# Duy1230/Map-Reduced-Approach-for-Vietnamese-Long-Document-Summarization

Hardware: AMD Instinct MI355X
Metric: map-phase chunks/sec (2k-tok chunk, 256-tok summary) at 1/2/4/8 MI355X (higher is better)
Workload: dtype f16

## Files before the change

### include/mapsum.h

```cpp
#ifndef MAPSUM_H
#define MAPSUM_H

#include <stddef.h>
#include <stdint.h>

#ifdef __cplusplus
extern "C" {
#endif

#define MS_ABI_VERSION 3

#define MS_OK 0
#define MS_EIO -5
#define MS_ENOMEM -12
#define MS_EBUSY -16
#define MS_EINVAL -22
#define MS_ENOSPC -28

#define MS_FINISH_EOS 1
#define MS_FINISH_LENGTH 2
#define MS_FINISH_ERROR 3

#define MS_FLAG_IGNORE_EOS 1u

// ... 67 lines not shown
                     const void* host_blocks, int64_t n_bytes);
int ms_init_synthetic_q(ms_engine* e, uint64_t seed, float scale, float norm_jitter);

int ms_weight_regions(const ms_engine* e, void** ptrs, int64_t* bytes, int32_t cap);
int ms_quant_manifest(const ms_engine* e, int32_t* triples, int32_t cap);
int ms_declare_weight_q(ms_engine* e, int32_t tensor, int32_t layer, int32_t ggml_type);

int ms_submit(ms_engine* e, const int32_t* ids, int32_t n, int32_t num_predict,
              uint32_t flags, uint64_t tag);
#define MS_SAMPLE_MAX_TOPK 256
#define MS_SAMPLE_MAX_WINDOW 256
typedef struct ms_sampling {
  float temperature;
  int32_t top_k;
  float top_p;
  float min_p;
  float repeat_penalty;
  int32_t repeat_last_n;
  uint64_t seed;
} ms_sampling;
int ms_submit_sampled(ms_engine* e, const int32_t* ids, int32_t n, int32_t num_predict,
                      uint32_t flags, uint64_t tag, const ms_sampling* sp);
int ms_set_eos_ids(ms_engine* e, const int32_t* ids, int32_t n);
int ms_step(ms_engine* e);
int ms_poll(ms_engine* e, ms_result* out, int32_t cap);
int ms_pending(const ms_engine* e);
int ms_get_stats(const ms_engine* e, ms_stats* out);
int ms_reset_stats(ms_engine* e);
int ms_set_profiling(ms_engine* e, uint32_t class_mask);
int ms_trace_push(const char* name);
int ms_trace_pop(void);
int ms_synchronize(ms_engine* e);
int ms_set_persist(ms_engine* e, int32_t on);
#define MS_DBG_KPOOL 0
#define MS_DBG_VPOOL 1
#define MS_DBG_DECODE_LOGITS 2
#define MS_DBG_DECODE_X 3
#define MS_DBG_PREFILL_LOGITS 4
int ms_debug_read(ms_engine* e, int32_t which, int64_t offset, void* host, int64_t bytes);
int ms_debug_pk_stamps(uint64_t* out, int32_t n);
int ms_debug_a2_stamps(uint64_t* out, int32_t n);

int ms_forward(ms_engine* e, const int32_t* ids, int32_t n, int32_t n_layers_run,
               float* hidden_out, float* logits_out);
int ms_forward_packed(ms_engine* e, const int32_t* ids, const int32_t* lens, int32_t n_seqs,
                      int32_t n_layers_run, float* hidden_out, float* logits_out);
int ms_submit_forced(ms_engine* e, const int32_t* ids, int32_t n, const int32_t* forced,
                     int32_t n_forced, int32_t num_predict, uint32_t flags, uint64_t tag);

#define MS_EPI_STORE_F16 0
#define MS_EPI_ADD_F32 1
#define MS_EPI_SWIGLU 2
#define MS_EPI_STORE_F32 3
#define MS_EPI_ARGMAX 5
int ms_op_gemm(const void* A, const void* W, void* out, int32_t M, int32_t N, int32_t K,
               int32_t ldo, int32_t epilogue, void* stream);
int ms_op_gemm_resid(const void* A, const void* W, float* x, void* xg_out, const void* gamma, float* ssq_out,
                     int32_t M, int32_t N, int32_t K, void* stream);
int ms_gemm_resid_tiles(int32_t M, int32_t N);
int ms_set_gemm_variant(int32_t variant);
int ms_set_qgemv_gs(int32_t on);
int ms_set_attn_tuning(int32_t combine_grp, int32_t order);
int ms_set_dgemm_kh(int32_t kh);
int ms_set_dgemm_wn(int32_t wn);
int64_t ms_op_gemv_workspace(int32_t M, int32_t N, int32_t K);
int ms_op_gemv(const void* X, const void* W, void* out, int32_t M, int32_t N, int32_t K,
// ... 36 lines not shown
```

### map-reduced-approach-for-vietnamese-long-document-summarization_amd/csrc/engine.cpp

```cpp
#include <hip/hip_runtime.h>

#include <algorithm>
#include <cmath>
#include <cstddef>
#include <cstdio>
#include <cstdlib>
#include <cstring>
#include <deque>
#include <array>
#include <functional>
#include <map>
#include <tuple>
#include <memory>
#include <stdexcept>
#include <string>
#include <vector>

#if MS_HAVE_ROCTX
#include <rocprofiler-sdk-roctx/roctx.h>
#else
static inline int roctxRangePushA(const char*) { return 0; }
static inline int roctxRangePop() { return 0; }
#endif

// ... 142 lines not shown
  }
  bool large(int) const { return large_engine && (!has_quant || cfg.max_batch >= qlarge_min); }
  bool qd(const QSlot* q, int M, int N, int K, int S, int epi) const {
    if (!qdgemm_mode || !q || !q->ready()) return false;
    const QMat& m = q->m;
    const bool q4 = m.type0 == MS_QT_Q4_K && (m.n < 2 || m.type1 == MS_QT_Q4_K) && (m.n < 3 || m.type2 == MS_QT_Q4_K);
    return (q4 || qdgemm_mode == 2) && qdgemm_supported(M, N, K, S, epi, m);
  }
  bool row_groups(int B) const { return !large(B) && B > kMaxGemvRows; }
  int qsplit = 4;
  bool attn_slabs = true;
  RowScale cur_rs{};
  int32_t* args_d = nullptr;
  int32_t* args_h = nullptr;
  size_t args_cap = 0;
  struct Ctx {
    hipStream_t stream = nullptr;
    float* x = nullptr;
    float* ssq = nullptr;
    f16_t *xb = nullptr, *qkv = nullptr, *attn = nullptr, *hbuf = nullptr;
    float* logits = nullptr;
    int32_t* ids_out_d = nullptr;
    int32_t* args_d = nullptr;
    int32_t* args_h = nullptr;
    size_t args_cap = 0;
    hipEvent_t ev_a = nullptr, ev_b = nullptr;
  } cp, cd;
  bool overlap = false;
  void use(const Ctx& c) {
    stream = c.stream; x = c.x; ssq = c.ssq; xb = c.xb; qkv = c.qkv; attn = c.attn; hbuf = c.hbuf;
    logits = c.logits; ids_out_d = c.ids_out_d; args_d = c.args_d; args_h = c.args_h;
    args_cap = c.args_cap; ev_a = c.ev_a; ev_b = c.ev_b;
  }
  std::vector<uint8_t> stop_set;
  std::deque<std::unique_ptr<Seq>> waiting;
  std::vector<std::unique_ptr<Seq>> running;
  std::vector<std::unique_ptr<Seq>> done, polled;
  ms_stats stats{};
  uint32_t prof_mask = 0;
  std::vector<std::pair<int, int>> ev_pending;
  size_t ev_used = 0;
  hipEvent_t ev_a = nullptr, ev_b = nullptr;
  std::map<std::tuple<int, int, int, int>, std::pair<hipGraphExec_t, uint64_t>> decode_graphs;
  uint64_t graph_clock = 0;
  static constexpr size_t kMaxGraphs = 64;
  int graph_steps = 16;
  bool use_graphs = true;
  int32_t* ids_host = nullptr;
  int32_t* first_host = nullptr;
  int32_t* ids_ring_d = nullptr;
  static constexpr int kMaxRun = 64;
  int max_run = kMaxRun;
  SampleSlot* samp_d = nullptr;
  SampleSlot* samp_h = nullptr;
  std::vector<uint8_t> slot_sampled;

  template <class T>
  T* dalloc(size_t n, bool zero = false) {
    void* p = nullptr;
    if (n == 0) n = 1;
    hipError_t e = hipMalloc(&p, n * sizeof(T));
    if (e != hipSuccess)
      throw MsError(MS_ENOMEM, "hipMalloc(" + std::to_string(n * sizeof(T)) + " B) failed: " +
                                   hipGetErrorString(e));
    allocs.push_back(p);
    if (zero) HIP_OK(hipMemset(p, 0, n * sizeof(T)));
// ... 193 lines not shown
      ga.tok_pos = tok_pos;
      ga.tok_slot = tok_slot;
      ga.cos_tab = cos_tab;
      ga.sin_tab = sin_tab;
      ga.kv = kv;
      ga.Hq = Hq;
      ga.Hk = Hk;
      ga.rs = rs_attn;
      proj(&Q[QS_QKV], xb, Ly.wqkv, qkv, B, QKVN, H, QKVN, MS_GEMV_EPI_ROPE_KV, &ga, K_GEMV);
      qa = DecodeQKV{qkv, nullptr, 0, cos_tab, sin_tab, RowScale{}};
    }
    attn_decode(qa, kv, da);
    resid_update(&Q[QS_O], attn, Ly.wo, B, Hq * D, split_o, dsplit_o, Ly.ffn_norm, dwn_o);
    const RowScale rs_ffn = cur_rs;
    const f16_t* g_next = l + 1 < L ? layers[l + 1].attn_norm : final_norm;
    if (large(B)) {
      prof_begin(K_GEMV);
      if (qd(&Q[QS_GU], B, 2 * F, H, 1, MS_GEMV_EPI_SWIGLU))
        launch_qdgemm(xb, Q[QS_GU].m, hbuf, B, 2 * F, H, 1, F, MS_GEMV_EPI_SWIGLU, stream, &rs_ffn);
      else if (qdf(B, 2 * F, H, 1, MS_GEMV_EPI_SWIGLU))
        launch_qdgemm_f16(xb, Ly.wgu, hbuf, B, 2 * F, H, 1, F, MS_GEMV_EPI_SWIGLU, stream, &rs_ffn);
      else
        launch_dgemm(xb, Ly.wgu, hbuf, B, 2 * F, H, 1, F, MS_GEMV_EPI_SWIGLU, stream, &rs_ffn, dgemm_kh);
      prof_end(K_GEMV);
    } else {
      GemvArgs gg{};
      gg.rs = rs_ffn;
      proj(&Q[QS_GU], xb, Ly.wgu, hbuf, B, 2 * F, H, F, MS_GEMV_EPI_SWIGLU, &gg, K_GEMV, sizeof(f16_t));
    }
    resid_update(&Q[QS_DOWN], hbuf, Ly.wdown, B, F, split_down, dsplit_down, g_next, dwn_down);
  }

  void run_layer(int l, int T, bool decode, const int32_t* tok_pos, const int32_t* tok_slot,
                 const PrefillAttnArgs& pa, const DecodeAttnArgs& da, bool tail = true) {
    if (decode && fused_decode(T)) {
      run_layer_fused_decode(l, T, tok_pos, tok_slot, da);
      return;
    }
    const Layer& Ly = layers[l];
    const int kc = decode ? K_GEMV : K_GEMM;
    const RowScale rs_attn = cur_rs;
    KVView kv = kv_layer(l);
    gemm_or_gemv(xb, Ly.wqkv, qkv, T, QKVN, H, QKVN, MS_EPI_STORE_F16, decode, kc, &rs_attn);
    prof_begin(K_MISC);
    launch_rope_kv(qkv, T, Hq, Hk, tok_pos, tok_slot, cos_tab, sin_tab, kv, stream, decode || !pa.cos_tab);
    prof_end(K_MISC);
    if (decode) {
      attn_decode(DecodeQKV{qkv, nullptr, 0, cos_tab, sin_tab, RowScale{}}, kv, da);
    } else {
      prof_begin(K_ATTN_PREFILL);
      launch_attn_prefill(qkv, attn, Hq, Hk, kv, pa, stream);
      prof_end(K_ATTN_PREFILL);
    }
    const f16_t* g_next = l + 1 < L ? layers[l + 1].attn_norm : final_norm;
    if (decode) {
      gemm_or_gemv(attn, Ly.wo, x, T, H, Hq * D, H, MS_EPI_ADD_F32, decode, kc);
      norm_input(Ly.ffn_norm, T);
    } else {
      prefill_resid(attn, Ly.wo, T, Hq * D, Ly.ffn_norm);
    }
    const RowScale rs_ffn = cur_rs;
    gemm_or_gemv(xb, Ly.wgu, hbuf, T, 2 * F, H, F, MS_EPI_SWIGLU, decode, kc, &rs_ffn);
    if (decode) {
      gemm_or_gemv(hbuf, Ly.wdown, x, T, H, F, H, MS_EPI_ADD_F32, decode, kc);
      if (tail) norm_input(g_next, T);
    } else if (tail) {
      prefill_resid(hbuf, Ly.wdown, T, F, g_next);
    } else {
      gemm_or_gemv(hbuf, Ly.wdown, x, T, H, F, H, MS_EPI_ADD_F32, decode, kc);
    }
  }

  bool prefill_resid_ok(int T) const {
    const int tiles = gemm_resid_tiles(T, H);
    return tiles <= kGemmRsTiles && gemm_rs_tiles_ok(T, QKVN, tiles) && gemm_rs_tiles_ok(T, 2 * F, tiles);
  }
  void prefill_resid(const f16_t* X, const f16_t* W, int T, int K, const f16_t* g_next) {
    if (!prefill_resid_ok(T)) {
      gemm_or_gemv(X, W, x, T, H, K, H, MS_EPI_ADD_F32, false, K_GEMM);
      norm_input(g_next, T);
      return;
    }
    GemmResid gr{g_next, xb, ssq};
    prof_begin(K_GEMM);
    launch_gemm(X, W, x, T, H, K, H, MS_EPI_ADD_F32, stream, nullptr, &gr);
    prof_end(K_GEMM);
    cur_rs = make_row_scale(ssq, gemm_resid_tiles(T, H), H, cfg.norm_eps);
  }

  void norm_input(const f16_t* w, int T, const int32_t* row_idx = nullptr) {
    prof_begin(K_MISC);
    launch_rmsnorm(x, w, xb, ssq, T, H, row_idx, stream);
    prof_end(K_MISC);
    cur_rs = norm_rs();
  }

  std::vector<std::array<int32_t, 3>> quant_manifest;
  void note_quant(int tensor, int layer, int type) {
    for (auto& q : quant_manifest)
      if (q[0] == tensor && q[1] == layer) { q[2] = type; return; }
    quant_manifest.push_back({tensor, layer, type});
  }
  std::vector<std::pair<void*, size_t>> weight_regions() const {
    std::vector<std::pair<void*, size_t>> r;
    const size_t H2 = (size_t)H * 2;
    r.push_back({embed, (size_t)V * H2});
    if (!cfg.tie_embeddings) r.push_back({lm_head, (size_t)V * H2});
    r.push_back({final_norm, H2});
    for (const Layer& Ly : layers) {
      r.push_back({Ly.attn_norm, H2});
      r.push_back({Ly.ffn_norm, H2});
      r.push_back({Ly.wqkv, (size_t)QKVN * H2});
      r.push_back({Ly.wo, (size_t)Hq * D * H2});
      r.push_back({Ly.wgu, (size_t)2 * F * H2});
      r.push_back({Ly.wdown, (size_t)F * H2});
    }
    auto qs = [&](const QSlot& q) {
      const uint8_t* b[3] = {q.m.base0, q.m.base1, q.m.base2};
      for (int i = 0; i < 3; ++i)
        if (b[i]) r.push_back({(void*)b[i], q.bytes[i]});
    };
    qs(lmq);
    for (const auto& l : lq)
      for (const QSlot& q : l) qs(q);
    return r;
// ... 127 lines not shown
      Ly.ffn_norm = E.dalloc<f16_t>(E.H);
      Ly.wqkv = E.dalloc<f16_t>((size_t)E.QKVN * E.H);
      Ly.wo = E.dalloc<f16_t>((size_t)E.H * E.Hq * E.D);
      Ly.wgu = E.dalloc<f16_t>((size_t)2 * E.F * E.H);
      Ly.wdown = E.dalloc<f16_t>((size_t)E.H * E.F);
    }
    std::vector<float> cs, sn;
    rope_tables(*cfg, cfg->max_ctx, cs, sn);
    E.cos_tab = E.dalloc<float>(cs.size());
    E.sin_tab = E.dalloc<float>(sn.size());
    HIP_OK(hipMemcpy(E.cos_tab, cs.data(), cs.size() * 4, hipMemcpyHostToDevice));
    HIP_OK(hipMemcpy(E.sin_tab, sn.data(), sn.size() * 4, hipMemcpyHostToDevice));
    E.layer_kv_elems = (size_t)E.n_pages * E.Hk * kPage * E.D;
    E.kpool = E.dalloc<f16_t>(E.layer_kv_elems * E.L, true);
    E.vpool = E.dalloc<f16_t>(E.layer_kv_elems * E.L, true);
    HIP_OK(hipHostMalloc((void**)&E.bt_h, (size_t)cfg->max_batch * E.max_pages * sizeof(int32_t),
                         hipHostMallocDefault));
    std::memset(E.bt_h, 0, (size_t)cfg->max_batch * E.max_pages * sizeof(int32_t));
    E.bt_d = E.dalloc<int32_t>((size_t)cfg->max_batch * E.max_pages, true);
    for (int p = E.n_pages - 1; p >= 0; --p) E.free_pages.push_back(p);
    for (int s = cfg->max_batch - 1; s >= 0; --s) E.free_slots.push_back(s);
    const size_t T = E.Tmax;
    for (ms_engine::Ctx* c : {&E.cp, &E.cd}) {
      const size_t R = c == &E.cp ? T : (size_t)cfg->max_batch;
      c->x = E.dalloc<float>(R * E.H);
      c->ssq = E.dalloc<float>(std::max(R * kGemmRsTiles, (size_t)256 * cfg->max_batch), true);
      c->xb = E.dalloc<f16_t>(R * E.H);
      c->qkv = E.dalloc<f16_t>(R * E.QKVN);
      c->attn = E.dalloc<f16_t>(R * E.Hq * E.D);
      c->hbuf = E.dalloc<f16_t>(R * E.F);
      c->logits = E.dalloc<float>((size_t)cfg->max_batch * E.V);
      c->ids_out_d = E.dalloc<int32_t>(cfg->max_batch);
    }
    const int Md = std::min(cfg->max_batch, 64);
    size_t gws = 0;
    const int shapes[5][2] = {{E.QKVN, E.H}, {E.H, E.Hq * E.D}, {2 * E.F, E.H}, {E.H, E.F}, {E.V, E.H}};
    for (auto& sh : shapes) gws = std::max(gws, gemv_workspace_bytes(Md, sh[0], sh[1]));
    E.gemv_ws = E.dalloc<char>(gws, true);
    E.attn_ppb = attn_decode2_ppb(cfg->max_batch, E.Hk, cfg->max_ctx);
    E.attn_v2 = cfg->max_batch <= 16;
    if (const char* v = getenv("MS_ATTN_V2")) E.attn_v2 = atoi(v) != 0;
    if (const char* v = getenv("MS_ATTN_TICKET")) E.attn_ticket = atoi(v) != 0;
    E.attn_cnt = E.dalloc<unsigned>((size_t)cfg->max_batch * E.Hk, true);
    const int ws_ctx = (cfg->max_ctx + 255) / 256 * 256;
    E.attn_ws = (float*)E.dalloc<char>(std::max(attn_decode_workspace_bytes(cfg->max_batch, E.Hq, ws_ctx),
                                                attn_decode2_workspace_bytes(cfg->max_batch, E.Hq, ws_ctx,
                                                                             E.attn_ppb)),
                                       true);
    E.slabs = E.dalloc<float>((size_t)ms_engine::kMaxSplit * std::min(std::max(cfg->max_batch, 64), 256) *
                              std::max(E.QKVN, E.H));
    if (const char* v = getenv("MS_SPLIT_QKV")) E.split_qkv = atoi(v);
    if (const char* v = getenv("MS_ATTN_SLABS")) E.attn_slabs = atoi(v) != 0;
    if (const char* v = getenv("MS_SPLIT_O")) E.split_o = atoi(v);
    if (const char* v = getenv("MS_SPLIT_DOWN")) E.split_down = atoi(v);
    if (const char* v = getenv("MS_DGEMM_MIN")) E.dgemm_min = atoi(v);
    E.large_engine = cfg->max_batch >= E.dgemm_min;
    if (const char* v = getenv("MS_QLARGE_MIN")) E.qlarge_min = atoi(v);
    if (const char* v = getenv("MS_QDGEMM")) E.qdgemm_mode = atoi(v);
    if (const char* v = getenv("MS_LM_GEMM_MIN")) E.lm_gemm_min = atoi(v);
    E.dgemm_kh = cfg->max_batch <= 128 && E.H % 128 == 0 ? dgemm_kh_setting() : 1;
    if (const char* v = getenv("MS_QDF_MIN")) E.qdf_min = atoi(v);
    if (E.qdf_min > 0 && cfg->max_batch >= E.qdf_min) {
      E.dsplit_qkv = 3;
      E.dsplit_down = 4;
    }
    if (const char* v = getenv("MS_DSPLIT_QKV")) E.dsplit_qkv = atoi(v);
// ... 520 lines not shown
  const size_t o_ids = a.size();
  for (Seq* s : batch) a.insert(a.end(), s->prompt.begin(), s->prompt.end());
  const size_t o_pos = a.size();
  for (Seq* s : batch)
    for (int i = 0; i < (int)s->prompt.size(); ++i) a.push_back(s->len + i);
  const size_t o_slot = a.size();
  for (Seq* s : batch)
    for (int i = 0; i < (int)s->prompt.size(); ++i) a.push_back(s->slot);
  const size_t o_qstart = a.size();
  {
    int q = 0;
    for (Seq* s : batch) { a.push_back(q); q += (int)s->prompt.size(); }
  }
  const size_t o_qlen = a.size();
  for (Seq* s : batch) a.push_back((int)s->prompt.size());
  const size_t o_kvlen = a.size();
  for (Seq* s : batch) a.push_back(s->len + (int)s->prompt.size());
  const size_t o_sslot = a.size();
  for (Seq* s : batch) a.push_back(s->slot);
  const size_t o_last = a.size();
  {
    int q = 0;
    for (Seq* s : batch) { q += (int)s->prompt.size(); a.push_back(q - 1); }
  }
  std::vector<std::pair<int, int32_t>> qb;
  for (int i = 0; i < S; ++i) {
    const int n = (int)batch[i]->prompt.size();
    for (int b = 0; b < (n + kPrefillQRows - 1) / kPrefillQRows; ++b)
      qb.push_back({batch[i]->len + b * kPrefillQRows, (i << 16) | b});
  }
  std::stable_sort(qb.begin(), qb.end(), [](auto& x, auto& y) { return x.first > y.first; });
  const size_t o_qblk = a.size();
  for (auto& p : qb) a.push_back(p.second);
  int32_t* d = E.upload_args(a);

  PrefillAttnArgs pa;
  pa.seq_qstart = d + o_qstart;
  pa.seq_qlen = d + o_qlen;
  pa.seq_kvlen = d + o_kvlen;
  pa.seq_slot = d + o_sslot;
  pa.qblk = d + o_qblk;
  pa.n_qblk = (int)qb.size();
  pa.cos_tab = E.cos_tab;
  pa.sin_tab = E.sin_tab;
  DecodeAttnArgs da{};

  E.prof_begin(K_MISC);
  launch_embed(d + o_ids, T, E.embed, E.H, E.x, E.stream);
  E.prof_end(K_MISC);
  E.norm_input(E.layers[0].attn_norm, T);
  for (int l = 0; l < n_layers_run; ++l)
    E.run_layer(l, T, false, d + o_pos, d + o_slot, pa, da, l + 1 < E.L || logits_all);
  HIP_OK(hipGetLastError());
  if (n_layers_run < E.L) return;
  if (!logits_all && !first_ids) return;
  if (logits_all) {
    launch_gemm(E.xb, E.lm_head, logits_all, T, E.V, E.H, E.V, MS_EPI_STORE_F32, E.stream, &E.cur_rs);
    return;
  }
  E.norm_input(E.final_norm, S, d + o_last);
  for (int r0 = 0; r0 < S; r0 += ms_engine::kMaxGemvRows) {
    const int rows = std::min(S - r0, (int)ms_engine::kMaxGemvRows);
    const RowScale rs = make_row_scale(E.ssq + r0, 1, E.H, E.cfg.norm_eps);
    E.gemm_or_gemv(E.xb + (size_t)r0 * E.H, E.lm_head, E.logits + (size_t)r0 * E.V, rows, E.V, E.H, E.V,
                   MS_EPI_STORE_F32, true, K_LMHEAD, &rs);
  }
  bool samp = false;
  for (Seq* s : batch) samp = samp || s->sampled;
  E.prof_begin(K_MISC);
  if (samp) {
    SampleArgs sa{};
    sa.logits = E.logits;
    sa.ldl = E.V;
    sa.n = E.V;
    sa.slots = E.samp_d;
    sa.row_slot = d + o_sslot;
    sa.ids_out = E.ids_out_d;
    launch_sample_rows(sa, S, E.stream);
  } else {
    launch_argmax(E.logits, S, E.V, E.ids_out_d, E.stream);
  }
  E.prof_end(K_MISC);
  HIP_OK(hipGetLastError());
  first_ids->resize(S);
  HIP_OK(hipMemcpyAsync(E.first_host, E.ids_out_d, S * sizeof(int32_t), hipMemcpyDeviceToHost, E.stream));
}

static void decode_head(ms_engine& E, int B, int32_t* d) {
  E.prof_begin(K_MISC);
  launch_embed(d, B, E.embed, E.H, E.x, E.stream, E.layers[0].attn_norm, E.xb, E.ssq);
  E.prof_end(K_MISC);
}

// ... 356 lines not shown
int ms_trace_pop(void) {
  roctxRangePop();
  return MS_OK;
}

int ms_get_stats(const ms_engine* e, ms_stats* out) {
  if (!e || !out) return MS_EINVAL;
  *out = e->stats;
  return MS_OK;
}

int ms_reset_stats(ms_engine* e) {
  if (!e) return MS_EINVAL;
  e->stats = ms_stats{};
  return MS_OK;
}

int ms_set_profiling(ms_engine* e, uint32_t mask) {
  if (!e) return MS_EINVAL;
  e->prof_mask = mask;
  return MS_OK;
}

int ms_set_persist(ms_engine* e, int32_t on) {
  if (!e) return MS_EINVAL;
  return guarded(e, [&]() -> int {
    HIP_OK(hipStreamSynchronize(e->cd.stream));
    e->persist = on != 0;
    e->drop_graphs();
    return (e->persist_ok ? 1 : 0);
  });
}

int ms_debug_read(ms_engine* e, int32_t which, int64_t offset, void* host, int64_t bytes) {
  if (!e || !host || offset < 0 || bytes < 0) return MS_EINVAL;
  return guarded(e, [&]() -> int {
    ms_engine& E = *e;
    const void* base = nullptr;
    size_t cap = 0;
    switch (which) {
      case MS_DBG_KPOOL: base = E.kpool; cap = E.layer_kv_elems * E.L * sizeof(f16_t); break;
      case MS_DBG_VPOOL: base = E.vpool; cap = E.layer_kv_elems * E.L * sizeof(f16_t); break;
      case MS_DBG_DECODE_LOGITS: base = E.cd.logits; cap = (size_t)E.cfg.max_batch * E.V * sizeof(float); break;
      case MS_DBG_DECODE_X: base = E.cd.x; cap = (size_t)E.cfg.max_batch * E.H * sizeof(float); break;
      case MS_DBG_PREFILL_LOGITS: base = E.cp.logits; cap = (size_t)E.cfg.max_batch * E.V * sizeof(float); break;
      default: REQUIRE(false, MS_EINVAL, "ms_debug_read: unknown buffer");
    }
    REQUIRE((size_t)offset + (size_t)bytes <= cap, MS_EINVAL, "ms_debug_read: range past the buffer");
    HIP_OK(hipStreamSynchronize(E.cd.stream));
    HIP_OK(hipStreamSynchronize(E.cp.stream));
    HIP_OK(hipMemcpy(host, (const char*)base + offset, (size_t)bytes, hipMemcpyDeviceToHost));
    return MS_OK;
  });
}

int ms_debug_pk_stamps(uint64_t* out, int32_t n) {
  if (!out || n < 0) return MS_EINVAL;
  ms::persist_stamps(reinterpret_cast<unsigned long long*>(out), n);
  return MS_OK;
}

int ms_debug_a2_stamps(uint64_t* out, int32_t n) {
  if (!out || n < 0) return MS_EINVAL;
  ms::attn2_stamps(reinterpret_cast<unsigned long long*>(out), n);
  return MS_OK;
}
// ... 381 lines not shown
```

### map-reduced-approach-for-vietnamese-long-document-summarization_amd/csrc/k_misc.hip

```cpp
#include "gemv_common.h"

namespace ms {

thread_local ProfEvents* g_prof = nullptr;

__global__ __launch_bounds__(256) void embed_kernel(const int32_t* __restrict__ ids,
                                                    const f16_t* __restrict__ emb, int H,
                                                    float* __restrict__ x, const f16_t* __restrict__ gamma,
                                                    f16_t* __restrict__ xg, float* __restrict__ ssq) {
  __shared__ float red[4];
  const int t = blockIdx.x;
  const f16_t* row = emb + (size_t)ids[t] * H;
  float* xo = x + (size_t)t * H;
  float ss = 0.f;
  for (int c = threadIdx.x; c < H / 8; c += blockDim.x) {
    uint4 v = *(const uint4*)(row + c * 8);
    const uint32_t w[4] = {v.x, v.y, v.z, v.w};
    float4 a, b;
    a.x = h_lo(w[0]); a.y = h_hi(w[0]);
    a.z = h_lo(w[1]); a.w = h_hi(w[1]);
    b.x = h_lo(w[2]); b.y = h_hi(w[2]);
    b.z = h_lo(w[3]); b.w = h_hi(w[3]);
    *(float4*)(xo + c * 8) = a;
    *(float4*)(xo + c * 8 + 4) = b;
// ... 144 lines not shown
  float4 v[8];
  float ss = 0.f;
#pragma unroll
  for (int k = 0; k < 8; ++k) {
    const int c = min(threadIdx.x + k * 256, n4 - 1);
    v[k] = *(const float4*)(xr + c * 4);
    if (threadIdx.x + k * 256 < n4) ss += v[k].x * v[k].x + v[k].y * v[k].y + v[k].z * v[k].z + v[k].w * v[k].w;
  }
  f16_t* yr = y + (size_t)r * H;
#pragma unroll
  for (int k = 0; k < 8; ++k) {
    const int c = threadIdx.x + k * 256;
    if (c >= n4) break;
    uint2 wv = *(const uint2*)(w + c * 4);
    float g0 = h_lo(wv.x), g1 = h_hi(wv.x);
    float g2 = h_lo(wv.y), g3 = h_hi(wv.y);
    uint2 o;
    o.x = pack2h(v[k].x * g0 * kXgScale, v[k].y * g1 * kXgScale);
    o.y = pack2h(v[k].z * g2 * kXgScale, v[k].w * g3 * kXgScale);
    *(uint2*)(yr + c * 4) = o;
  }
  ss = wave_sum(ss);
  if ((threadIdx.x & 63) == 0) red[threadIdx.x >> 6] = ss;
  __syncthreads();
  if (threadIdx.x == 0) ssq[r] = ((red[0] + red[1]) + red[2]) + red[3];
}

void launch_rmsnorm(const float* x, const f16_t* w, f16_t* y, float* ssq, int rows, int H,
                    const int32_t* row_idx, hipStream_t s) {
  if (rows <= 0) return;
  MS_LAUNCH(rmsnorm_kernel, dim3(rows), dim3(256), 0, s, x, w, y, ssq, H, row_idx);
}

template <int S>
__global__ __launch_bounds__(256) void residual_rmsnorm_kernel(float* __restrict__ x,
                                                               const float* __restrict__ slabs,
                                                               int rows,
                                                               const f16_t* __restrict__ w,
                                                               f16_t* __restrict__ y,
                                                               float* __restrict__ ssq, int H) {
  constexpr int KMAX = 3;
  __shared__ float red[4];
  const int r = blockIdx.x;
  float* xr = x + (size_t)r * H;
  const int n4 = H / 4;
  const size_t slab = (size_t)rows * H;
  typedef uint32_t u32x2 __attribute__((ext_vector_type(2)));
  f32x4 v[KMAX], p[KMAX][S > 0 ? S : 1];
  u32x2 wv[KMAX];
#pragma unroll
  for (int k = 0; k < KMAX; ++k) {
    const int c = min((int)threadIdx.x + k * 256, n4 - 1);
    v[k] = *(const f32x4*)(xr + c * 4);
    wv[k] = *(const u32x2*)(w + c * 4);
#pragma unroll
    for (int q = 0; q < S; ++q) p[k][q] = *(const f32x4*)(slabs + q * slab + (size_t)r * H + c * 4);
  }
  __builtin_amdgcn_sched_barrier(0);
#pragma unroll
  for (int k = 0; k < KMAX; ++k) {
    asm volatile("" : "+v"(v[k]));
    asm volatile("" : "+v"(wv[k]));
#pragma unroll
    for (int q = 0; q < S; ++q) asm volatile("" : "+v"(p[k][q]));
  }
  if constexpr (S > 0) {
// ... 233 lines not shown
```

### map-reduced-approach-for-vietnamese-long-document-summarization_amd/csrc/kernels.h

```cpp
#pragma once
#include "common.h"

namespace ms {

struct KVView {
  f16_t* k;
  f16_t* v;
  const int32_t* block_table;
  int32_t max_pages;
  int32_t n_kv_heads;
  int32_t slot_major;
};

constexpr int kPrefillQRows = 128;
struct PrefillAttnArgs {
  const int32_t* seq_qstart;
  const int32_t* seq_qlen;
  const int32_t* seq_kvlen;
  const int32_t* seq_slot;
  const int32_t* qblk;
  int32_t n_qblk;
  const float* cos_tab;
  const float* sin_tab;
};

struct DecodeAttnArgs {
  const int32_t* seq_len;
  const int32_t* seq_slot;
  int32_t B;
  int32_t max_len;
  int32_t ppw;
};

struct RowScale {
  const float* ssq;
  int tiles, H;
  float eps;
  float inv_h;
};
inline RowScale make_row_scale(const float* ssq, int tiles, int H, float eps) {
  return RowScale{ssq, tiles, H, eps, 1.0f / (float)H};
}
constexpr float kXgScale = 0.0625f, kXgUnscale = 16.0f;
__device__ __forceinline__ float rs_rinv(float sum, const RowScale& rs) {
  return __builtin_amdgcn_rsqf(__fmaf_rn(sum, rs.inv_h, rs.eps)) * kXgUnscale;
}

void launch_embed(const int32_t* ids, int T, const f16_t* emb, int H, float* x, hipStream_t s,
                  const f16_t* gamma = nullptr, f16_t* xg = nullptr, float* ssq = nullptr);
void launch_decode_advance(int32_t* args, const int32_t* ids_out, int32_t* ring, int B, int V,
                           hipStream_t s);
void launch_decode_tail(const void* partials, int tiles, int32_t* args, int32_t* ids_out, int32_t* ring, int B,
                        int V, const f16_t* emb, int H, float* x, const f16_t* gamma, f16_t* xg, float* ssq,
                        hipStream_t s);
void launch_rmsnorm(const float* x, const f16_t* w, f16_t* y, float* ssq, int rows, int H,
                    const int32_t* row_idx, hipStream_t s);
void launch_rope_kv(f16_t* qkv, int T, int Hq, int Hk, const int32_t* tok_pos,
                    const int32_t* tok_slot, const float* cos_tab, const float* sin_tab,
                    KVView kv, hipStream_t s, bool rope_q = true);
void launch_argmax(const float* logits, int rows, int n, int32_t* out, hipStream_t s);

constexpr int kSampleMaxTopK = 256, kSampleMaxWindow = 256;
constexpr int kSampleMaxN = 131072;
struct SampleParams {
  float temperature;
  int32_t top_k;
  float top_p, min_p, repeat_penalty;
  int32_t repeat_last_n;
  uint64_t seed;
};
struct SampleSlot {
  SampleParams p;
  int32_t wcount;
  int32_t step;
  int32_t ring[kSampleMaxWindow];
};
struct SampleArgs {
  const float* logits;
  int64_t ldl;
  int n;
  const SampleParams* params;
  const int32_t* win;
  const int32_t* win_len;
  const int32_t* steps;
  SampleSlot* slots;
  const int32_t* row_slot;
  int32_t* ids_out;
  int32_t* cand_ids;
  float* cand_p;
// ... 192 lines not shown
```

### map-reduced-approach-for-vietnamese-long-document-summarization_amd/mapsum/_lib.py

```python
from __future__ import annotations

import ctypes as C
import os

_HERE = os.path.dirname(os.path.abspath(__file__))
LIB_PATH = os.environ.get("MAPSUM_LIB") or os.path.join(_HERE, "libmapsum.so")

MS_ABI_VERSION = 3
MS_OK, MS_EIO, MS_ENOMEM, MS_EBUSY, MS_EINVAL, MS_ENOSPC = 0, -5, -12, -16, -22, -28
MS_FINISH_EOS, MS_FINISH_LENGTH, MS_FINISH_ERROR = 1, 2, 3
MS_FLAG_IGNORE_EOS = 1
(MS_T_EMBED, MS_T_ATTN_NORM, MS_T_WQ, MS_T_WK, MS_T_WV, MS_T_WO, MS_T_FFN_NORM, MS_T_WGATE,
 MS_T_WUP, MS_T_WDOWN, MS_T_FINAL_NORM, MS_T_LM_HEAD) = range(12)
MS_EPI_STORE_F16, MS_EPI_ADD_F32, MS_EPI_SWIGLU, MS_EPI_STORE_F32 = range(4)
MS_EPI_ARGMAX = 5
GEMM_DEFAULT = 4
MS_GGML_Q4_K, MS_GGML_Q6_K = 12, 14
K_GEMM, K_ATTN_PREFILL, K_GEMV, K_ATTN_DECODE, K_LMHEAD, K_MISC, K_PERSIST = range(7)
MS_DBG_KPOOL, MS_DBG_VPOOL, MS_DBG_DECODE_LOGITS, MS_DBG_DECODE_X, MS_DBG_PREFILL_LOGITS = range(5)
MS_SAMPLE_MAX_TOPK, MS_SAMPLE_MAX_WINDOW = 256, 256

EXPORTED = (
    "ms_create", "ms_destroy", "ms_last_error", "ms_load_weight", "ms_init_synthetic",
    "ms_load_weight_q", "ms_init_synthetic_q", "ms_op_dequant", "ms_op_quant_rows", "ms_op_qgemv", "ms_op_qgemv_split", "ms_op_qdgemm",
    "ms_submit", "ms_step", "ms_poll", "ms_pending", "ms_get_stats", "ms_reset_stats",
    "ms_set_profiling", "ms_synchronize", "ms_forward", "ms_op_gemm", "ms_op_gemv_workspace",
    "ms_op_gemv", "ms_op_gemv_tuned", "ms_op_gemv_split", "ms_op_dgemm", "ms_op_residual_rmsnorm", "ms_op_rmsnorm",
    "ms_op_argmax", "ms_op_argmax_partials", "ms_set_gemm_variant", "ms_set_qgemv_gs", "ms_set_attn_tuning", "ms_set_dgemm_kh", "ms_set_dgemm_wn",
    "ms_weight_regions", "ms_quant_manifest", "ms_declare_weight_q",
    "ms_forward_packed", "ms_submit_forced", "ms_set_eos_ids", "ms_op_gemv_strided",
    "ms_op_gemv_resid", "ms_op_set_row_scale", "ms_op_gemm_resid", "ms_gemm_resid_tiles",
    "ms_trace_push", "ms_trace_pop", "ms_debug_a2_stamps", "ms_set_persist", "ms_debug_read", "ms_debug_pk_stamps",
    "ms_submit_sampled", "ms_op_sample",
)


class MsConfig(C.Structure):
    _fields_ = [("abi_version", C.c_int32),
                ("n_layers", C.c_int32), ("hidden", C.c_int32), ("n_heads", C.c_int32),
                ("n_kv_heads", C.c_int32), ("head_dim", C.c_int32), ("ffn", C.c_int32),
                ("vocab", C.c_int32),
                ("rope_theta", C.c_float), ("rope_factor", C.c_float),
                ("rope_low_freq_factor", C.c_float), ("rope_high_freq_factor", C.c_float),
                ("rope_orig_ctx", C.c_int32), ("norm_eps", C.c_float), ("tie_embeddings", C.c_int32),
                ("device", C.c_int32), ("max_batch", C.c_int32), ("max_ctx", C.c_int32),
                ("max_prefill_tokens", C.c_int32), ("n_pages", C.c_int32), ("n_eos", C.c_int32),
                ("eos_ids", C.c_int32 * 8)]


class MsSampling(C.Structure):
    _fields_ = [("temperature", C.c_float), ("top_k", C.c_int32), ("top_p", C.c_float),
                ("min_p", C.c_float), ("repeat_penalty", C.c_float), ("repeat_last_n", C.c_int32),
                ("seed", C.c_uint64)]


class MsResult(C.Structure):
    _fields_ = [("tag", C.c_uint64), ("ids", C.POINTER(C.c_int32)), ("n_ids", C.c_int32),
                ("finish_reason", C.c_int32), ("n_prompt", C.c_int32), ("_pad", C.c_int32)]


class MsStats(C.Structure):
    _fields_ = [("prefill_tokens", C.c_int64), ("decode_tokens", C.c_int64),
                ("prefill_passes", C.c_int64), ("decode_steps", C.c_int64), ("finished", C.c_int64),
                ("prefill_ms", C.c_double), ("decode_ms", C.c_double),
                ("kernel_ms", C.c_double * 8), ("kernel_launches", C.c_int64 * 8),
                ("decode_kv_tokens", C.c_int64), ("graphs_built", C.c_int64),
# ... 41 lines not shown
        "ms_reset_stats": (i32, [vp]),
        "ms_set_profiling": (i32, [vp, u32]),
        "ms_synchronize": (i32, [vp]),
        "ms_forward": (i32, [vp, pi32, i32, i32, vp, vp]),
        "ms_forward_packed": (i32, [vp, pi32, pi32, i32, i32, vp, vp]),
        "ms_set_eos_ids": (i32, [vp, pi32, i32]),
        "ms_op_gemv_strided": (i32, [vp, vp, vp, i32, i32, i32, i32, i32, i32, vp]),
        "ms_op_gemv_resid": (i32, [vp, vp, vp, vp, vp, vp, i32, i32, i32, i32, vp]),
        "ms_op_set_row_scale": (i32, [vp, i32, i32, C.c_float]),
        "ms_op_gemm_resid": (i32, [vp, vp, vp, vp, vp, vp, i32, i32, i32, vp]),
        "ms_gemm_resid_tiles": (i32, [i32, i32]),
        "ms_submit_forced": (i32, [vp, pi32, i32, pi32, i32, i32, u32, u64]),
        "ms_op_gemm": (i32, [vp, vp, vp, i32, i32, i32, i32, i32, vp]),
        "ms_op_gemv_workspace": (i64, [i32, i32, i32]),
        "ms_op_gemv": (i32, [vp, vp, vp, i32, i32, i32, i32, i32, vp, vp]),
        "ms_op_gemv_tuned": (i32, [vp, vp, vp, i32, i32, i32, i32, i32, vp, i32, vp]),
        "ms_op_gemv_split": (i32, [vp, vp, vp, i32, i32, i32, i32, i32, vp]),
        "ms_op_dgemm": (i32, [vp, vp, vp, i32, i32, i32, i32, i32, i32, vp]),
        "ms_op_residual_rmsnorm": (i32, [vp, vp, i32, vp, vp, vp, i32, i32, vp]),
        "ms_op_rmsnorm": (i32, [vp, vp, vp, vp, i32, i32, vp, vp]),
        "ms_set_gemm_variant": (i32, [i32]),
        "ms_set_qgemv_gs": (i32, [i32]),
        "ms_set_attn_tuning": (i32, [i32, i32]),
        "ms_set_dgemm_kh": (i32, [i32]),
        "ms_set_dgemm_wn": (i32, [i32]),
        "ms_op_argmax": (i32, [vp, i32, i32, vp, vp]),
        "ms_op_argmax_partials": (i32, [vp, i32, i32, vp, vp]),
        "ms_weight_regions": (i32, [vp, C.POINTER(vp), C.POINTER(i64), i32]),
        "ms_quant_manifest": (i32, [vp, pi32, i32]),
        "ms_declare_weight_q": (i32, [vp, i32, i32, i32]),
        "ms_trace_push": (i32, [C.c_char_p]),
        "ms_trace_pop": (i32, []),
        "ms_set_persist": (i32, [vp, i32]),
        "ms_debug_read": (i32, [vp, i32, i64, vp, i64]),
        "ms_debug_pk_stamps": (i32, [vp, i32]),
        "ms_debug_a2_stamps": (i32, [vp, i32]),
    }
    for name, (res, args) in sig.items():
        if ab and not hasattr(lib, name):
            continue
        fn = getattr(lib, name)
        fn.restype = res
        fn.argtypes = args
    return lib


def check(rc: int, handle=None, what: str = "") -> int:
    if rc < 0:
        msg = load().ms_last_error(handle)
        raise RuntimeError(f"libmapsum {what} failed ({rc}): {msg.decode() if msg else ''}")
    return rc


class trace:

    def __init__(self, name: str):
        self.name = name.encode()
        self.lib = None

    def __enter__(self):
        try:
            lib = load()
            if hasattr(lib, "ms_trace_push"):
                lib.ms_trace_push(self.name)
                self.lib = lib
        except (OSError, RuntimeError):
# ... 8 lines not shown
```

### map-reduced-approach-for-vietnamese-long-document-summarization_amd/mapsum/engine.py

```python
from __future__ import annotations

import ctypes as C
import math
from dataclasses import dataclass, replace

import numpy as np

from . import _lib as L
from .config import ModelConfig


@dataclass
class Result:
    tag: int
    ids: list
    finish: str
    n_prompt: int


SAMPLING_OPTIONS = ("temperature", "top_k", "top_p", "min_p", "repeat_penalty", "repeat_last_n", "seed")


@dataclass(frozen=True)
class Sampling:
# ... 291 lines not shown
        lens = np.ascontiguousarray([len(p) for p in prompts], dtype=np.int32)
        n = a.size
        nl = cfg.n_layers if n_layers is None else n_layers
        hid = np.empty((n, cfg.hidden), np.float32) if hidden else None
        lg = np.empty((n, cfg.vocab), np.float32) if logits else None
        p32 = C.POINTER(C.c_int32)
        self._chk(self.lib.ms_forward_packed(self.h, a.ctypes.data_as(p32), lens.ctypes.data_as(p32), lens.size,
                                             nl, hid.ctypes.data if hid is not None else None,
                                             lg.ctypes.data if lg is not None else None), "ms_forward_packed")
        return hid, lg

    def set_profiling(self, mask: int):
        self._chk(self.lib.ms_set_profiling(self.h, mask), "ms_set_profiling")

    def reset_stats(self):
        self._chk(self.lib.ms_reset_stats(self.h), "ms_reset_stats")

    def synchronize(self):
        self._chk(self.lib.ms_synchronize(self.h), "ms_synchronize")

    def stats(self) -> dict:
        s = L.MsStats()
        self._chk(self.lib.ms_get_stats(self.h, C.byref(s)), "ms_get_stats")
        return {"prefill_tokens": s.prefill_tokens, "decode_tokens": s.decode_tokens,
                "prefill_passes": s.prefill_passes, "decode_steps": s.decode_steps,
                "finished": s.finished, "prefill_ms": s.prefill_ms, "decode_ms": s.decode_ms,
                "kernel_ms": list(s.kernel_ms), "kernel_launches": list(s.kernel_launches),
                "decode_kv_tokens": s.decode_kv_tokens, "graphs_built": s.graphs_built,
                "persist_fallbacks": s.persist_fallbacks, "persist_steps": s.persist_steps}

    def set_persist(self, on: bool) -> bool:
        return bool(self._chk(self.lib.ms_set_persist(self.h, 1 if on else 0), "ms_set_persist"))

    def debug_read(self, which: int, offset: int, nbytes: int) -> np.ndarray:
        out = np.empty(nbytes, np.uint8)
        self._chk(self.lib.ms_debug_read(self.h, which, offset, out.ctypes.data, nbytes), "ms_debug_read")
        return out
```

Baseline: 12.90.

## Compute only last-token rows through final prefill layer's Q, attention and FFN

In the last transformer layer of a prefill pass, K/V are still projected and written to the cache for every token. The residual stream, normalized input and norm statistics are then gathered down to each sequence's last row. Only those rows go through the Q projection, attention (with a compact query-block layout), output projection and FFN, because only the final-token hidden state feeds the LM head. This removes about one layer of full-length GEMM and attention work per prefill, at the cost of a gather kernel, extra compact buffers and a more involved layer path controlled by an env/API toggle that defaults on.

```diff
diff --git a/include/mapsum.h b/include/mapsum.h
--- a/include/mapsum.h
+++ b/include/mapsum.h
@@ -123,6 +123,7 @@
 int ms_trace_pop(void);
 int ms_synchronize(ms_engine* e);
 int ms_set_persist(ms_engine* e, int32_t on);
+int ms_set_prefill_last_rows(ms_engine* e, int32_t on);
 #define MS_DBG_KPOOL 0
 #define MS_DBG_VPOOL 1
 #define MS_DBG_DECODE_LOGITS 2
diff --git a/map-reduced-approach-for-vietnamese-long-document-summarization_amd/csrc/engine.cpp b/map-reduced-approach-for-vietnamese-long-document-summarization_amd/csrc/engine.cpp
--- a/map-reduced-approach-for-vietnamese-long-document-summarization_amd/csrc/engine.cpp
+++ b/map-reduced-approach-for-vietnamese-long-document-summarization_amd/csrc/engine.cpp
@@ -198,6 +198,15 @@
     logits = c.logits; ids_out_d = c.ids_out_d; args_d = c.args_d; args_h = c.args_h;
     args_cap = c.args_cap; ev_a = c.ev_a; ev_b = c.ev_b;
   }
+  bool last_rows = true;
+  float* lr_x = nullptr;
+  f16_t* lr_xb = nullptr;
+  float* lr_ssq = nullptr;
+  struct LastRows {
+    int S;
+    const int32_t* row_idx;
+    PrefillAttnArgs pa;
+  };
   std::vector<uint8_t> stop_set;
   std::deque<std::unique_ptr<Seq>> waiting;
   std::vector<std::unique_ptr<Seq>> running;
@@ -457,7 +466,8 @@
   }
 
   void run_layer(int l, int T, bool decode, const int32_t* tok_pos, const int32_t* tok_slot,
-                 const PrefillAttnArgs& pa, const DecodeAttnArgs& da, bool tail = true) {
+                 const PrefillAttnArgs& pa, const DecodeAttnArgs& da, bool tail = true,
+                 const LastRows* lr = nullptr) {
     if (decode && fused_decode(T)) {
       run_layer_fused_decode(l, T, tok_pos, tok_slot, da);
       return;
@@ -466,15 +476,44 @@
     const int kc = decode ? K_GEMV : K_GEMM;
     const RowScale rs_attn = cur_rs;
     KVView kv = kv_layer(l);
-    gemm_or_gemv(xb, Ly.wqkv, qkv, T, QKVN, H, QKVN, MS_EPI_STORE_F16, decode, kc, &rs_attn);
-    prof_begin(K_MISC);
-    launch_rope_kv(qkv, T, Hq, Hk, tok_pos, tok_slot, cos_tab, sin_tab, kv, stream, decode || !pa.cos_tab);
-    prof_end(K_MISC);
+    struct Rows {
+      ms_engine& E;
+      float *x, *ssq;
+      f16_t* xb;
+      ~Rows() { E.x = x; E.ssq = ssq; E.xb = xb; }
+    } packed_rows{*this, x, ssq, xb};
+    const PrefillAttnArgs* ap = &pa;
+    if (lr && !decode) {
+      const int QD = Hq * D;
+      REQUIRE(lr->S >= 1 && lr->S <= cfg.max_batch && lr->S <= T && rs_attn.ssq && rs_attn.tiles >= 1 &&
+                  rs_attn.tiles <= kGemmRsTiles,
+              MS_EINVAL, "last-rows prefill: rows or statistics tiles exceed the compact buffers");
+      gemm_or_gemv(xb, Ly.wqkv + (size_t)QD * H, qkv + QD, T, QKVN - QD, H, QKVN, MS_EPI_STORE_F16, false, kc,
+                   &rs_attn);
+      prof_begin(K_MISC);
+      launch_rope_kv(qkv, T, Hq, Hk, tok_pos, tok_slot, cos_tab, sin_tab, kv, stream, false);
+      prof_end(K_MISC);
+      prof_begin(K_MISC);
+      launch_gather_rows(x, xb, rs_attn.ssq, lr->row_idx, lr->S, T, H, rs_attn.tiles, lr_x, lr_xb, lr_ssq, stream);
+      prof_end(K_MISC);
+      x = lr_x;
+      xb = lr_xb;
+      ssq = lr_ssq;
+      T = lr->S;
+      cur_rs = make_row_scale(lr_ssq, rs_attn.tiles, H, cfg.norm_eps);
+      gemm_or_gemv(xb, Ly.wqkv, qkv, T, QD, H, QKVN, MS_EPI_STORE_F16, false, kc, &cur_rs);
+      ap = &lr->pa;
+    } else {
+      gemm_or_gemv(xb, Ly.wqkv, qkv, T, QKVN, H, QKVN, MS_EPI_STORE_F16, decode, kc, &rs_attn);
+      prof_begin(K_MISC);
+      launch_rope_kv(qkv, T, Hq, Hk, tok_pos, tok_slot, cos_tab, sin_tab, kv, stream, decode || !pa.cos_tab);
+      prof_end(K_MISC);
+    }
     if (decode) {
       attn_decode(DecodeQKV{qkv, nullptr, 0, cos_tab, sin_tab, RowScale{}}, kv, da);
     } else {
       prof_begin(K_ATTN_PREFILL);
-      launch_attn_prefill(qkv, attn, Hq, Hk, kv, pa, stream);
+      launch_attn_prefill(qkv, attn, Hq, Hk, kv, *ap, stream);
       prof_end(K_ATTN_PREFILL);
     }
     const f16_t* g_next = l + 1 < L ? layers[l + 1].attn_norm : final_norm;
@@ -513,9 +552,9 @@
     cur_rs = make_row_scale(ssq, gemm_resid_tiles(T, H), H, cfg.norm_eps);
   }
 
-  void norm_input(const f16_t* w, int T, const int32_t* row_idx = nullptr) {
+  void norm_input(const f16_t* w, int T, const int32_t* row_idx = nullptr, const float* src = nullptr) {
     prof_begin(K_MISC);
-    launch_rmsnorm(x, w, xb, ssq, T, H, row_idx, stream);
+    launch_rmsnorm(src ? src : x, w, xb, ssq, T, H, row_idx, stream);
     prof_end(K_MISC);
     cur_rs = norm_rs();
   }
@@ -709,6 +748,10 @@
       c->logits = E.dalloc<float>((size_t)cfg->max_batch * E.V);
       c->ids_out_d = E.dalloc<int32_t>(cfg->max_batch);
     }
+    E.lr_x = E.dalloc<float>((size_t)cfg->max_batch * E.H);
+    E.lr_xb = E.dalloc<f16_t>((size_t)cfg->max_batch * E.H);
+    E.lr_ssq = E.dalloc<float>((size_t)kGemmRsTiles * cfg->max_batch, true);
+    if (const char* v = getenv("MS_PREFILL_LAST_ROWS")) E.last_rows = atoi(v) != 0;
     const int Md = std::min(cfg->max_batch, 64);
     size_t gws = 0;
     const int shapes[5][2] = {{E.QKVN, E.H}, {E.H, E.Hq * E.D}, {2 * E.F, E.H}, {E.H, E.F}, {E.V, E.H}};
@@ -1295,6 +1338,16 @@
   std::stable_sort(qb.begin(), qb.end(), [](auto& x, auto& y) { return x.first > y.first; });
   const size_t o_qblk = a.size();
   for (auto& p : qb) a.push_back(p.second);
+  const bool last_rows = E.last_rows && n_layers_run == E.L && !logits_all && first_ids;
+  const size_t o_lr = a.size();
+  if (last_rows) {
+    for (int i = 0; i < S; ++i) a.push_back(i);
+    for (int i = 0; i < S; ++i) a.push_back(1);
+    std::vector<std::pair<int, int32_t>> qc;
+    for (int i = 0; i < S; ++i) qc.push_back({batch[i]->len + (int)batch[i]->prompt.size(), i << 16});
+    std::stable_sort(qc.begin(), qc.end(), [](auto& x, auto& y) { return x.first > y.first; });
+    for (auto& p : qc) a.push_back(p.second);
+  }
   int32_t* d = E.upload_args(a);
 
   PrefillAttnArgs pa;
@@ -1312,8 +1365,14 @@
   launch_embed(d + o_ids, T, E.embed, E.H, E.x, E.stream);
   E.prof_end(K_MISC);
   E.norm_input(E.layers[0].attn_norm, T);
+  ms_engine::LastRows lr{S, d + o_last, pa};
+  lr.pa.seq_qstart = d + o_lr;
+  lr.pa.seq_qlen = d + o_lr + S;
+  lr.pa.qblk = d + o_lr + 2 * S;
+  lr.pa.n_qblk = S;
   for (int l = 0; l < n_layers_run; ++l)
-    E.run_layer(l, T, false, d + o_pos, d + o_slot, pa, da, l + 1 < E.L || logits_all);
+    E.run_layer(l, T, false, d + o_pos, d + o_slot, pa, da, l + 1 < E.L || logits_all,
+                last_rows && l + 1 == E.L ? &lr : nullptr);
   HIP_OK(hipGetLastError());
   if (n_layers_run < E.L) return;
   if (!logits_all && !first_ids) return;
@@ -1321,7 +1380,8 @@
     launch_gemm(E.xb, E.lm_head, logits_all, T, E.V, E.H, E.V, MS_EPI_STORE_F32, E.stream, &E.cur_rs);
     return;
   }
-  E.norm_input(E.final_norm, S, d + o_last);
+  if (last_rows) E.norm_input(E.final_norm, S, nullptr, E.lr_x);
+  else E.norm_input(E.final_norm, S, d + o_last);
   for (int r0 = 0; r0 < S; r0 += ms_engine::kMaxGemvRows) {
     const int rows = std::min(S - r0, (int)ms_engine::kMaxGemvRows);
     const RowScale rs = make_row_scale(E.ssq + r0, 1, E.H, E.cfg.norm_eps);
@@ -1744,6 +1804,12 @@
   });
 }
 
+int ms_set_prefill_last_rows(ms_engine* e, int32_t on) {
+  if (!e) return MS_EINVAL;
+  e->last_rows = on != 0;
+  return MS_OK;
+}
+
 int ms_debug_read(ms_engine* e, int32_t which, int64_t offset, void* host, int64_t bytes) {
   if (!e || !host || offset < 0 || bytes < 0) return MS_EINVAL;
   return guarded(e, [&]() -> int {
diff --git a/map-reduced-approach-for-vietnamese-long-document-summarization_amd/csrc/k_misc.hip b/map-reduced-approach-for-vietnamese-long-document-summarization_amd/csrc/k_misc.hip
--- a/map-reduced-approach-for-vietnamese-long-document-summarization_amd/csrc/k_misc.hip
+++ b/map-reduced-approach-for-vietnamese-long-document-summarization_amd/csrc/k_misc.hip
@@ -200,6 +200,28 @@
   MS_LAUNCH(rmsnorm_kernel, dim3(rows), dim3(256), 0, s, x, w, y, ssq, H, row_idx);
 }
 
+__global__ __launch_bounds__(256) void gather_rows_kernel(const float* __restrict__ x, const f16_t* __restrict__ xg,
+                                                          const float* __restrict__ ssq,
+                                                          const int32_t* __restrict__ row_idx, int H, int tiles,
+                                                          int src_rows, float* __restrict__ xo,
+                                                          f16_t* __restrict__ xgo, float* __restrict__ ssqo) {
+  const int r = blockIdx.x, rows = gridDim.x;
+  const int src = min(max(row_idx[r], 0), src_rows - 1);
+  const float4* xs = (const float4*)(x + (size_t)src * H);
+  float4* xd = (float4*)(xo + (size_t)r * H);
+  for (int c = threadIdx.x; c < H / 4; c += blockDim.x) xd[c] = xs[c];
+  const uint4* gs = (const uint4*)(xg + (size_t)src * H);
+  uint4* gd = (uint4*)(xgo + (size_t)r * H);
+  for (int c = threadIdx.x; c < H / 8; c += blockDim.x) gd[c] = gs[c];
+  for (int t = threadIdx.x; t < tiles; t += blockDim.x) ssqo[(size_t)t * rows + r] = ssq[(size_t)t * src_rows + src];
+}
+
+void launch_gather_rows(const float* x, const f16_t* xg, const float* ssq, const int32_t* row_idx, int rows,
+                        int src_rows, int H, int tiles, float* xo, f16_t* xgo, float* ssqo, hipStream_t s) {
+  if (rows <= 0 || src_rows <= 0) return;
+  MS_LAUNCH(gather_rows_kernel, dim3(rows), dim3(256), 0, s, x, xg, ssq, row_idx, H, tiles, src_rows, xo, xgo, ssqo);
+}
+
 template <int S>
 __global__ __launch_bounds__(256) void residual_rmsnorm_kernel(float* __restrict__ x,
                                                                const float* __restrict__ slabs,
diff --git a/map-reduced-approach-for-vietnamese-long-document-summarization_amd/csrc/kernels.h b/map-reduced-approach-for-vietnamese-long-document-summarization_amd/csrc/kernels.h
--- a/map-reduced-approach-for-vietnamese-long-document-summarization_amd/csrc/kernels.h
+++ b/map-reduced-approach-for-vietnamese-long-document-summarization_amd/csrc/kernels.h
@@ -55,6 +55,8 @@
                         hipStream_t s);
 void launch_rmsnorm(const float* x, const f16_t* w, f16_t* y, float* ssq, int rows, int H,
                     const int32_t* row_idx, hipStream_t s);
+void launch_gather_rows(const float* x, const f16_t* xg, const float* ssq, const int32_t* row_idx, int rows,
+                        int src_rows, int H, int tiles, float* xo, f16_t* xgo, float* ssqo, hipStream_t s);
 void launch_rope_kv(f16_t* qkv, int T, int Hq, int Hk, const int32_t* tok_pos,
                     const int32_t* tok_slot, const float* cos_tab, const float* sin_tab,
                     KVView kv, hipStream_t s, bool rope_q = true);
diff --git a/map-reduced-approach-for-vietnamese-long-document-summarization_amd/mapsum/_lib.py b/map-reduced-approach-for-vietnamese-long-document-summarization_amd/mapsum/_lib.py
--- a/map-reduced-approach-for-vietnamese-long-document-summarization_amd/mapsum/_lib.py
+++ b/map-reduced-approach-for-vietnamese-long-document-summarization_amd/mapsum/_lib.py
@@ -31,7 +31,7 @@
     "ms_forward_packed", "ms_submit_forced", "ms_set_eos_ids", "ms_op_gemv_strided",
     "ms_op_gemv_resid", "ms_op_set_row_scale", "ms_op_gemm_resid", "ms_gemm_resid_tiles",
     "ms_trace_push", "ms_trace_pop", "ms_debug_a2_stamps", "ms_set_persist", "ms_debug_read", "ms_debug_pk_stamps",
-    "ms_submit_sampled", "ms_op_sample",
+    "ms_submit_sampled", "ms_op_sample", "ms_set_prefill_last_rows",
 )
 
 
@@ -139,6 +139,7 @@
         "ms_trace_push": (i32, [C.c_char_p]),
         "ms_trace_pop": (i32, []),
         "ms_set_persist": (i32, [vp, i32]),
+        "ms_set_prefill_last_rows": (i32, [vp, i32]),
         "ms_debug_read": (i32, [vp, i32, i64, vp, i64]),
         "ms_debug_pk_stamps": (i32, [vp, i32]),
         "ms_debug_a2_stamps": (i32, [vp, i32]),
diff --git a/map-reduced-approach-for-vietnamese-long-document-summarization_amd/mapsum/engine.py b/map-reduced-approach-for-vietnamese-long-document-summarization_amd/mapsum/engine.py
--- a/map-reduced-approach-for-vietnamese-long-document-summarization_amd/mapsum/engine.py
+++ b/map-reduced-approach-for-vietnamese-long-document-summarization_amd/mapsum/engine.py
@@ -347,6 +347,9 @@
     def set_persist(self, on: bool) -> bool:
         return bool(self._chk(self.lib.ms_set_persist(self.h, 1 if on else 0), "ms_set_persist"))
 
+    def set_prefill_last_rows(self, on: bool):
+        self._chk(self.lib.ms_set_prefill_last_rows(self.h, 1 if on else 0), "ms_set_prefill_last_rows")
+
     def debug_read(self, which: int, offset: int, nbytes: int) -> np.ndarray:
         out = np.empty(nbytes, np.uint8)
         self._chk(self.lib.ms_debug_read(self.h, which, offset, out.ctypes.data, nbytes), "ms_debug_read")
```

New measurement: 12.94 (median of 6 runs). No clear change (+0.3%).
